# qdrant/quantization

Hardware: AMD Instinct MI355X
Metric: scored vectors/sec, 10Mx768 u8 dot (higher is better)
Workload: dtype u8; 1 GPU; 10000000 x 768 store: f32 U[0,1) -> scalar u8 (dot); per step: encode_query + score_all over the shard; quantizer=u8, rows_per_gpu=10000000, dim=768, distance=dot, exchange=scores, gather_group=1, launch=single rank, world_size_seen=1, encode_ahead=False, total_rows=10000000, queries=16

## Files before the change

quantization_amd/csrc/common.cpp:

```cpp
#include "common.hpp"

#include <sys/stat.h>

#include <cerrno>
#include <cmath>
#include <cstdlib>
#include <algorithm>
#include <atomic>
#include <fstream>
#include <mutex>
#include <vector>

namespace qamd {

static thread_local std::string g_last_error;
static thread_local int g_device = 0;

std::string &last_error() { return g_last_error; }

qamd_status fail(qamd_status st, const char *fmt, ...) {
    char buf[1024];
    va_list ap;
    va_start(ap, fmt);
    vsnprintf(buf, sizeof buf, fmt, ap);
    va_end(ap);
    g_last_error = buf;
    return st;
}

int current_device() { return g_device; }

int device_count() {
    static std::atomic<int> cached{-1};
    int n = cached.load(std::memory_order_relaxed);
    if (n > 0) return n;
    n = 0;
    if (hipGetDeviceCount(&n) != hipSuccess || n <= 0) {
        (void)hipGetLastError();
        return 0;
    }
    cached.store(n, std::memory_order_relaxed);
    return n;
}

DeviceGuard::DeviceGuard(int device) {
    const int n = device_count();
    if (n <= 0) {
        st_ = fail(QAMD_ERR_DEVICE, "no HIP device is visible; this library has no CPU fallback");
        return;
    }
    if (device < 0 || device >= n) {
        st_ = fail(QAMD_ERR_ARGUMENTS, "device %d out of range (have %d)", device, n);
        return;
    }
    hipError_t e = hipGetDevice(&prev_);
    if (e == hipSuccess && prev_ != device) {
        e = hipSetDevice(device);
        switched_ = e == hipSuccess;
    }
    if (e != hipSuccess) st_ = fail(QAMD_ERR_DEVICE, "cannot select device %d: %s", device, hipGetErrorString(e));
}

DeviceGuard::~DeviceGuard() {
    if (switched_) (void)hipSetDevice(prev_);
}

qamd_status DevBuf::alloc(size_t n, bool zero) {
    release();
    if (n == 0) n = 16;
    QAMD_HIP(hipMalloc(&ptr, n));
    bytes = n;
    if (zero) {
        QAMD_HIP(hipMemsetAsync(ptr, 0, n, nullptr));
        QAMD_HIP(hipStreamSynchronize(nullptr));
    }
    return QAMD_OK;
}

qamd_status DevBuf::alloc_zero_tail(size_t n, size_t keep) {
    QAMD_TRY(alloc(n, false));
    if (keep < bytes) {
        QAMD_HIP(hipMemsetAsync(static_cast<char *>(ptr) + keep, 0, bytes - keep, nullptr));
        QAMD_HIP(hipStreamSynchronize(nullptr));
    }
    return QAMD_OK;
}

void DevBuf::release() {
    if (ptr) (void)hipFree(ptr);
    ptr = nullptr;
    bytes = 0;
}

qamd_status grow_copy(const DevBuf &old, size_t n, size_t keep, DevBuf &out) {
    if (keep > n || keep > old.bytes) return fail(QAMD_ERR_ARGUMENTS, "grow_copy: keeps %zu of %zu bytes in %zu", keep, old.bytes, n);
    QAMD_TRY(out.alloc_zero_tail(n, keep));
    if (keep) {
        QAMD_HIP(hipMemcpyAsync(out.ptr, old.ptr, keep, hipMemcpyDeviceToDevice, nullptr));
        QAMD_HIP(hipStreamSynchronize(nullptr));
    }
    return QAMD_OK;
}

namespace {
struct QueryBufCache {
    struct Entry { void *ptr; size_t bytes; int dev; };
    std::mutex m;
    std::vector<Entry> free_list;
};
QueryBufCache &query_cache() {
    static QueryBufCache *c = new QueryBufCache;
    return *c;
}
constexpr size_t kQueryCacheEntries = 64;
}

qamd_status query_buf_get(size_t bytes, DevBuf &out) {
    out.release();
    int dev = 0;
    QAMD_HIP(hipGetDevice(&dev));
    {
        QueryBufCache &c = query_cache();
        std::lock_guard<std::mutex> lk(c.m);
        for (size_t i = 0; i < c.free_list.size(); i++) {
            if (c.free_list[i].dev == dev && c.free_list[i].bytes == bytes) {
                out.ptr = c.free_list[i].ptr;
                out.bytes = bytes;
                c.free_list[i] = c.free_list.back();
                c.free_list.pop_back();
                return QAMD_OK;
            }
        }
    }
    return out.alloc(bytes, true);
}

void query_buf_put(DevBuf &buf, bool idle) {
    if (!buf.ptr) return;
    hipPointerAttribute_t attr{};
    if (idle && hipPointerGetAttributes(&attr, buf.ptr) == hipSuccess) {
        QueryBufCache &c = query_cache();
        std::lock_guard<std::mutex> lk(c.m);
        if (c.free_list.size() < kQueryCacheEntries) {
            c.free_list.push_back({buf.ptr, buf.bytes, attr.device});
            buf.ptr = nullptr;
            buf.bytes = 0;
            return;
        }
    } else if (idle) {
        (void)hipGetLastError();
    }
    buf.release();
}

qamd_status StreamBuf::alloc(size_t n, hipStream_t s, bool zero) {
    release();
    static std::once_flag once[64];
    int dev = 0;
    if (hipGetDevice(&dev) == hipSuccess && dev >= 0 && dev < 64) {
        std::call_once(once[dev], [dev] {
            hipMemPool_t pool = nullptr;
            if (hipDeviceGetDefaultMemPool(&pool, dev) == hipSuccess && pool) {
                uint64_t keep = ~0ull;
                (void)hipMemPoolSetAttribute(pool, hipMemPoolAttrReleaseThreshold, &keep);
            }
        });
    }
    if (n == 0) n = 16;
    stream = s;
    QAMD_HIP(hipMallocAsync(&ptr, n, s));
    bytes = n;
    if (zero) QAMD_HIP(hipMemsetAsync(ptr, 0, n, s));
    return QAMD_OK;
}

void StreamBuf::release() {
    if (ptr) (void)hipFreeAsync(ptr, stream);
    ptr = nullptr;
    bytes = 0;
}

ReadyEvent::~ReadyEvent() {
    if (ev) (void)hipEventDestroy(ev);
}

qamd_status ReadyEvent::record(hipStream_t s) {
    if (!ev) QAMD_HIP(hipEventCreateWithFlags(&ev, hipEventDisableTiming));
    QAMD_HIP(hipEventRecord(ev, s));
    stream = s;
    set = true;
    return QAMD_OK;
}

bool ReadyEvent::complete() const {
    if (!set || !ev) return true;
    if (hipEventQuery(ev) == hipSuccess) return true;
    (void)hipGetLastError();
    return false;
}

qamd_status ReadyEvent::wait(hipStream_t consumer) const {
    if (!set || consumer == stream) return QAMD_OK;
    hipStreamCaptureStatus cap = hipStreamCaptureStatusNone;
    if (hipStreamIsCapturing(consumer, &cap) != hipSuccess) (void)hipGetLastError();
    if (cap == hipStreamCaptureStatusNone) {
        if (hipEventQuery(ev) == hipSuccess) return QAMD_OK;
        (void)hipGetLastError();
    }
    QAMD_HIP(hipStreamWaitEvent(consumer, ev, 0));
    return QAMD_OK;
}

qamd_status copy_in(void *dev_dst, const void *src, qamd_mem src_mem, size_t bytes, hipStream_t s) {
    if (bytes == 0) return QAMD_OK;
    if (src_mem == QAMD_MEM_DEVICE) {
        QAMD_HIP(hipMemcpyAsync(dev_dst, src, bytes, hipMemcpyDeviceToDevice, s));
    } else {
        QAMD_HIP(hipMemcpyAsync(dev_dst, src, bytes, hipMemcpyHostToDevice, s));
        QAMD_HIP(hipStreamSynchronize(s));
    }
    return QAMD_OK;
}

qamd_status copy_out(void *dst, qamd_mem dst_mem, const void *dev_src, size_t bytes, hipStream_t s) {
    if (bytes == 0) return QAMD_OK;
    if (dst_mem == QAMD_MEM_DEVICE) {
        QAMD_HIP(hipMemcpyAsync(dst, dev_src, bytes, hipMemcpyDeviceToDevice, s));
    } else {
        QAMD_HIP(hipMemcpyAsync(dst, dev_src, bytes, hipMemcpyDeviceToHost, s));
        QAMD_HIP(hipStreamSynchronize(s));
    }
    return QAMD_OK;
}

qamd_status local_view(const void *src, qamd_mem mem, size_t bytes, DevBuf &stage, hipStream_t s, const void **out,
                       bool *staged) {
    *out = src;
    *staged = false;
    if (bytes == 0) return QAMD_OK;
    bool remote = false;
    if (mem == QAMD_MEM_DEVICE && device_count() > 1) {
        hipPointerAttribute_t attr{};
        int dev = 0;
        if (hipPointerGetAttributes(&attr, src) == hipSuccess && hipGetDevice(&dev) == hipSuccess)
            remote = attr.device != dev;
        else
            (void)hipGetLastError();
    }
    if (mem == QAMD_MEM_DEVICE && !remote) return QAMD_OK;
    if (stage.bytes < bytes) QAMD_TRY(stage.alloc(bytes));
    QAMD_HIP(hipMemcpyAsync(stage.ptr, src, bytes, mem == QAMD_MEM_HOST ? hipMemcpyHostToDevice : hipMemcpyDefault, s));
    if (mem == QAMD_MEM_HOST) QAMD_HIP(hipStreamSynchronize(s));
    *out = stage.ptr;
    *staged = true;
    return QAMD_OK;
}

namespace {

constexpr int kMaxDevices = 64;

struct ThreadWs {
    void *ptr = nullptr;
    size_t bytes = 0;
    hipEvent_t done = nullptr;
    bool in_flight = false;
    uint64_t tags[3] = {0, 0, 0};
};

struct ThreadState {
    HostScratch scratch;
    bool scratch_tried = false;
    hipEvent_t query_read = nullptr;
    bool query_pending = false;
    std::vector<ThreadWs> ws;

    ThreadWs &at(int dev, ThreadWsSlot slot) {
        const size_t need = (size_t)(dev + 1) * WS_SLOTS;
        if (ws.size() < need) ws.resize(need);
        return ws[(size_t)dev * WS_SLOTS + slot];
    }

    void release() {
        int prev = -1;
        const bool have_prev = hipGetDevice(&prev) == hipSuccess;
        bool moved = false;
        for (size_t i = 0; i < ws.size(); i++) {
            ThreadWs &w = ws[i];
            if (!w.ptr) continue;
            const int dev = (int)(i / WS_SLOTS);
            if (hipSetDevice(dev) == hipSuccess) {
                moved = true;
                (void)hipFree(w.ptr);
                if (w.done) (void)hipEventDestroy(w.done);
            }
            w = ThreadWs{};
        }
        ws.clear();
        if (moved && have_prev) (void)hipSetDevice(prev);
        if (query_pending && query_read) (void)hipEventSynchronize(query_read);
        if (query_read) (void)hipEventDestroy(query_read);
        query_read = nullptr;
        query_pending = false;
        if (scratch.host) (void)hipHostFree(scratch.host);
        scratch = HostScratch{};
        scratch_tried = false;
        (void)hipGetLastError();
    }

    ~ThreadState() { release(); }
};

ThreadState &thread_state() {
    static thread_local ThreadState st;
    return st;
}

}

HostScratch host_scratch() {
    ThreadState &ts = thread_state();
    if (!ts.scratch_tried) {
        ts.scratch_tried = true;
        void *p = nullptr, *d = nullptr;
        if (hipHostMalloc(&p, kHostScratchWords * 4, hipHostMallocMapped | hipHostMallocPortable) == hipSuccess) {
            if (hipHostGetDevicePointer(&d, p, 0) == hipSuccess) {
                ts.scratch.host = static_cast<uint32_t *>(p);
                ts.scratch.dev = static_cast<uint32_t *>(d);
            } else {
                (void)hipHostFree(p);
            }
        }
    }
    return ts.scratch;
}

float *host_query_acquire(size_t n_floats, const float **dev_view) {
    if (n_floats > kHostQueryWords) return nullptr;
    const HostScratch hs = host_scratch();
    if (!hs.host) return nullptr;
    ThreadState &ts = thread_state();
    if (ts.query_pending) {
        if (hipEventSynchronize(ts.query_read) != hipSuccess) return nullptr;
        ts.query_pending = false;
    }
    if (!ts.query_read && hipEventCreateWithFlags(&ts.query_read, hipEventDisableTiming) != hipSuccess) {
        ts.query_read = nullptr;
        return nullptr;
    }
    *dev_view = reinterpret_cast<const float *>(hs.dev + kHostQueryAt);
    return reinterpret_cast<float *>(hs.host + kHostQueryAt);
}

void host_query_release(hipStream_t s) {
    ThreadState &ts = thread_state();
    if (ts.query_read && hipEventRecord(ts.query_read, s) == hipSuccess) ts.query_pending = true;
}

qamd_status thread_ws_acquire(ThreadWsSlot slot, size_t bytes, hipStream_t s, void **out, uint64_t **tags) {
    int dev = 0;
    QAMD_HIP(hipGetDevice(&dev));
    if (dev < 0 || dev >= kMaxDevices) return fail(QAMD_ERR_DEVICE, "device index %d not supported", dev);
    ThreadWs &w = thread_state().at(dev, slot);
    if (bytes == 0) bytes = 16;
    if (w.bytes < bytes) {
        if (w.ptr) {
            (void)hipFree(w.ptr);
            w.ptr = nullptr;
        }
        w.bytes = 0;
        w.in_flight = false;
        w.tags[0] = w.tags[1] = w.tags[2] = 0;
        const size_t want = bytes + bytes / 4;
        QAMD_HIP(hipMalloc(&w.ptr, want));
        w.bytes = want;
    }
    hipStreamCaptureStatus cap = hipStreamCaptureStatusNone;
    if (w.in_flight && hipStreamIsCapturing(s, &cap) != hipSuccess) (void)hipGetLastError();
    if (w.in_flight && cap == hipStreamCaptureStatusNone) {
        const hipError_t q = hipEventQuery(w.done);
        if (q == hipErrorNotReady) {
            (void)hipGetLastError();
            QAMD_HIP(hipStreamWaitEvent(s, w.done, 0));
        } else if (q != hipSuccess) {
            return fail(QAMD_ERR_DEVICE, "workspace hand-off: hipEventQuery failed: %s", hipGetErrorString(q));
        } else {
            w.in_flight = false;
        }
    }
    *out = w.ptr;
    if (tags) *tags = w.tags;
    return QAMD_OK;
}

void thread_ws_release(ThreadWsSlot slot, hipStream_t s, bool synced) {
    int dev = 0;
    if (hipGetDevice(&dev) != hipSuccess || dev < 0 || dev >= kMaxDevices) return;
    ThreadWs &w = thread_state().at(dev, slot);
    if (synced) {
        w.in_flight = false;
        return;
    }
    hipStreamCaptureStatus cap = hipStreamCaptureStatusNone;
    if (hipStreamIsCapturing(s, &cap) != hipSuccess) (void)hipGetLastError();
    if (cap != hipStreamCaptureStatusNone) return;
    w.in_flight = false;
    if (!w.done && hipEventCreateWithFlags(&w.done, hipEventDisableTiming) != hipSuccess) {
        w.done = nullptr;
        (void)hipGetLastError();
        (void)hipStreamSynchronize(s);
        return;
    }
    if (hipEventRecord(w.done, s) == hipSuccess) w.in_flight = true;
    else (void)hipStreamSynchronize(s);
}

void thread_release_all() { thread_state().release(); }

const DeviceInfo &device_info() {
    static DeviceInfo info[kMaxDevices];
    static std::atomic<uint64_t> known{0};
    int dev = 0;
    if (hipGetDevice(&dev) != hipSuccess || dev < 0 || dev >= kMaxDevices) dev = 0;
    if (!(known.load(std::memory_order_acquire) & (1ull << dev))) {
        hipDeviceProp_t p;
        if (hipGetDeviceProperties(&p, dev) == hipSuccess && p.multiProcessorCount > 0)
            info[dev].cu_count = p.multiProcessorCount;
        static const uint64_t forced = dev_env_u64("QAMD_DEV_CU_COUNT", 0);
        if (forced) info[dev].cu_count = (int)std::min<uint64_t>(forced, 1024);
        known.fetch_or(1ull << dev, std::memory_order_acq_rel);
    }
    return info[dev];
}

std::string json_f32(float v) {
    if (!std::isfinite(v)) return "null";
    std::string sign = std::signbit(v) ? "-" : "";
    if (v == 0.0f) return sign + "0.0";
    char buf[64];
    const double a = std::fabs((double)v);
    for (int p = 0; p <= 8; p++) {
        snprintf(buf, sizeof buf, "%.*e", p, a);
        if (strtof(buf, nullptr) == std::fabs(v)) break;
    }
    std::string digits;
    const char *e = strchr(buf, 'e');
    for (const char *c = buf; c < e; c++)
        if (*c != '.') digits += *c;
    const int exp10 = atoi(e + 1), length = (int)digits.size();
    const int kk = exp10 + 1, k = kk - length;
    if (0 <= k && kk <= 13) return sign + digits + std::string((size_t)k, '0') + ".0";
    if (0 < kk && kk <= 13) return sign + digits.substr(0, (size_t)kk) + "." + digits.substr((size_t)kk);
    if (-6 < kk && kk <= 0) return sign + "0." + std::string((size_t)(-kk), '0') + digits;
    if (length == 1) return sign + digits + "e" + std::to_string(kk - 1);
    return sign + digits.substr(0, 1) + "." + digits.substr(1) + "e" + std::to_string(kk - 1);
}

bool read_file(const char *path, std::string &out) {
    std::ifstream f(path, std::ios::binary);
    if (!f) return false;
    f.seekg(0, std::ios::end);
    std::streamoff n = f.tellg();
    f.seekg(0, std::ios::beg);
    out.resize((size_t)n);
    if (n > 0) f.read(&out[0], n);
    return bool(f) || f.eof();
}

static bool write_file(const char *path, const void *data, size_t bytes) {
    std::ofstream f(path, std::ios::binary | std::ios::trunc);
    if (!f) return false;
    if (bytes) f.write(static_cast<const char *>(data), (std::streamsize)bytes);
    f.flush();
    return bool(f);
}

static void make_parent_dirs(const char *path) {
    std::string p(path);
    size_t pos = p.find_last_of('/');
    if (pos == std::string::npos || pos == 0) return;
    std::string dir = p.substr(0, pos);
    for (size_t i = 1; i <= dir.size(); i++) {
        if (i == dir.size() || dir[i] == '/') {
            std::string sub = dir.substr(0, i);
            if (mkdir(sub.c_str(), 0777) != 0 && errno != EEXIST) return;
        }
    }
}

qamd_status save_file(const char *path, const void *data, size_t bytes) {
    make_parent_dirs(path);
    if (!write_file(path, data, bytes)) return fail(QAMD_ERR_IO, "cannot write %s", path);
    return QAMD_OK;
}

qamd_status load_rows_file(const char *data_path, uint64_t expected, std::string &bytes) {
    if (!read_file(data_path, bytes)) return fail(QAMD_ERR_IO, "cannot read %s", data_path);
    if (bytes.size() != expected)
        return fail(QAMD_ERR_IO, "Loaded storage size %zu is not equal to expected size %llu", bytes.size(),
                    (unsigned long long)expected);
    return QAMD_OK;
}

qamd_status count_mismatch(uint64_t got, uint64_t want) {
    return fail(QAMD_ERR_ARGUMENTS, "Vector count %llu does not match vector parameters count %llu", (unsigned long long)got,
// ... 99 lines not shown
```

quantization_amd/csrc/common.hpp:

```cpp
#pragma once

#include <hip/hip_runtime.h>

#include <algorithm>
#include <atomic>
#include <mutex>
#include <cstdarg>
#include <cstdint>
#include <cstdlib>
#include <cstdio>
#include <cstring>
#include <string>
#include <vector>

#include "json.hpp"

#include "../../include/quantization_amd.h"

namespace qamd {

std::string &last_error();
qamd_status fail(qamd_status st, const char *fmt, ...) __attribute__((format(printf, 2, 3)));

#define QAMD_HIP(expr)                                                                      \
    do {                                                                                    \
        hipError_t _e = (expr);                                                             \
        if (_e != hipSuccess)                                                               \
            return ::qamd::fail(QAMD_ERR_DEVICE, "%s failed: %s (%s:%d)", #expr,            \
                                hipGetErrorString(_e), __FILE__, __LINE__);                 \
    } while (0)

#define QAMD_TRY(expr)                    \
    do {                                  \
        qamd_status _s = (expr);          \
        if (_s != QAMD_OK) return _s;     \
    } while (0)

int current_device();
int device_count();

class DeviceGuard {
  public:
    explicit DeviceGuard(int device);
    ~DeviceGuard();
    DeviceGuard(const DeviceGuard &) = delete;
    DeviceGuard &operator=(const DeviceGuard &) = delete;
    qamd_status status() const { return st_; }

  private:
    int prev_ = -1;
    bool switched_ = false;
    qamd_status st_ = QAMD_OK;
};
#define QAMD_ON_DEVICE(dev)                  \
    ::qamd::DeviceGuard _qamd_dev_guard(dev); \
    QAMD_TRY(_qamd_dev_guard.status())

inline const char *dev_env(const char *name) {
#ifdef QAMD_DEV
    return getenv(name);
#else
    (void)name;
    return nullptr;
#endif
}
inline uint64_t dev_env_u64(const char *name, uint64_t dflt) {
    const char *e = dev_env(name);
    if (!e || !*e) return dflt;
    char *end = nullptr;
    const unsigned long long v = strtoull(e, &end, 10);
    return (*end == 0 && v > 0) ? (uint64_t)v : dflt;
}
inline uint64_t stage_bytes(uint64_t dflt) {
    static const uint64_t v = dev_env_u64("QAMD_DEV_STAGE_BYTES", 0);
    return v ? v : dflt;
}
inline bool host_whole_allowed() {
    static const bool on = [] { const char *e = dev_env("QAMD_DEV_HOST_WHOLE"); return !(e && e[0] == '0'); }();
    return on;
}
inline bool u8_packed_allowed() {
    static const bool on = [] { const char *e = dev_env("QAMD_DEV_U8_PACKED"); return !(e && e[0] == '0'); }();
    return on;
}
inline uint64_t pq_planar_max_rows() {
    static const uint64_t v = dev_env_u64("QAMD_DEV_PQ_PLANAR_ROWS", 1ull << 28);
    return v;
}
inline uint64_t pq_skew_max_rows() {
    static const uint64_t v = dev_env_u64("QAMD_DEV_PQ_SKEW_ROWS", 1ull << 30);
    return v;
}

class DeviceOnce {
  public:
    template <class F> qamd_status run(F &&setup) {
        int dev = 0;
        if (hipGetDevice(&dev) != hipSuccess || dev < 0 || dev > 63) return setup();
        const uint64_t bit = 1ull << dev;
        if (done_.load(std::memory_order_acquire) & bit) return QAMD_OK;
        std::lock_guard<std::mutex> g(mu_);
        if (done_.load(std::memory_order_relaxed) & bit) return QAMD_OK;
        const qamd_status st = setup();
        if (st == QAMD_OK) done_.fetch_or(bit, std::memory_order_release);
        return st;
    }

  private:
    std::atomic<uint64_t> done_{0};
    std::mutex mu_;
};
#define QAMD_LDS_OPT_IN(kernel, bytes)                                                                            \
    do {                                                                                                          \
        static ::qamd::DeviceOnce _qamd_once;                                                                     \
        QAMD_TRY(_qamd_once.run([]() -> qamd_status {                                                             \
            QAMD_HIP(hipFuncSetAttribute(reinterpret_cast<const void *>(kernel),                                  \
                                         hipFuncAttributeMaxDynamicSharedMemorySize, (int)(bytes)));              \
            return QAMD_OK;                                                                                       \
        }));                                                                                                      \
    } while (0)

struct DevBuf {
    void *ptr = nullptr;
    size_t bytes = 0;
    DevBuf() = default;
    DevBuf(const DevBuf &) = delete;
    DevBuf &operator=(const DevBuf &) = delete;
    DevBuf(DevBuf &&o) noexcept : ptr(o.ptr), bytes(o.bytes) { o.ptr = nullptr; o.bytes = 0; }
    DevBuf &operator=(DevBuf &&o) noexcept {
        if (this != &o) {
            release();
            ptr = o.ptr;
            bytes = o.bytes;
            o.ptr = nullptr;
            o.bytes = 0;
        }
        return *this;
    }
    ~DevBuf() { release(); }
    qamd_status alloc(size_t n, bool zero = false);
    qamd_status alloc_zero_tail(size_t n, size_t keep);
    void release();
    template <typename T> T *as() const { return static_cast<T *>(ptr); }
};

qamd_status grow_copy(const DevBuf &old, size_t n, size_t keep, DevBuf &out);

qamd_status query_buf_get(size_t bytes, DevBuf &out);
void query_buf_put(DevBuf &buf, bool idle);

inline hipStream_t as_stream(void *s) { return static_cast<hipStream_t>(s); }

struct StreamBuf {
    void *ptr = nullptr;
    size_t bytes = 0;
    hipStream_t stream = nullptr;
    StreamBuf() = default;
    StreamBuf(const StreamBuf &) = delete;
    StreamBuf &operator=(const StreamBuf &) = delete;
    ~StreamBuf() { release(); }
    qamd_status alloc(size_t n, hipStream_t s, bool zero = false);
    void release();
    template <typename T> T *as() const { return static_cast<T *>(ptr); }
};

struct ReadyEvent {
    hipEvent_t ev = nullptr;
    hipStream_t stream = nullptr;
    bool set = false;
    ReadyEvent() = default;
    ReadyEvent(const ReadyEvent &) = delete;
    ReadyEvent &operator=(const ReadyEvent &) = delete;
    ~ReadyEvent();
    qamd_status record(hipStream_t s);
    qamd_status wait(hipStream_t consumer) const;
    bool complete() const;
};

qamd_status copy_in(void *dev_dst, const void *src, qamd_mem src_mem, size_t bytes, hipStream_t s);
qamd_status copy_out(void *dst, qamd_mem dst_mem, const void *dev_src, size_t bytes, hipStream_t s);

constexpr size_t kHostQueryWords = 12288;
constexpr size_t kHostDoneAt = 2048 + 8;
constexpr size_t kHostQueryAt = 2048 + 16;
constexpr size_t kHostScratchWords = kHostQueryAt + kHostQueryWords;
struct HostScratch {
    uint32_t *host = nullptr;
    uint32_t *dev = nullptr;
};
HostScratch host_scratch();
float *host_query_acquire(size_t n_floats, const float **dev_view);
void host_query_release(hipStream_t s);

enum ThreadWsSlot { WS_SCORES = 0, WS_SELECT = 1, WS_PARTIAL = 2, WS_FUSED = 3, WS_SMALL = 4, WS_RESCORE = 5, WS_ROW_LUT = 6, WS_SLOTS = 7 };
qamd_status thread_ws_acquire(ThreadWsSlot slot, size_t bytes, hipStream_t s, void **out,
                              uint64_t **tags = nullptr);
void thread_ws_release(ThreadWsSlot slot, hipStream_t s, bool synced = false);
void thread_release_all();

qamd_status local_view(const void *src, qamd_mem mem, size_t bytes, DevBuf &stage, hipStream_t s, const void **out,
                       bool *staged);

template <class Consume>
qamd_status for_each_staged_piece(const float *batch, qamd_mem batch_mem, uint64_t n_rows, uint64_t dim, uint64_t piece_rows,
                                  DevBuf &stage, hipStream_t s, Consume &&consume) {
    for (uint64_t r = 0; r < n_rows; r += piece_rows) {
        const uint64_t nr = std::min(piece_rows, n_rows - r);
        const void *src = nullptr;
        bool staged = false;
        QAMD_TRY(local_view(batch + r * dim, batch_mem, nr * dim * 4, stage, s, &src, &staged));
        QAMD_TRY(consume(static_cast<const float *>(src), r, nr));
        if (staged) QAMD_HIP(hipStreamSynchronize(s));
    }
    return QAMD_OK;
}
qamd_status count_mismatch(uint64_t got, uint64_t want);
template <class Encoder> void abort_encoder(Encoder *e) {
    if (!e) return;
    DeviceGuard g(e->device);
    (void)hipStreamSynchronize(e->stream);
    delete e;
}
qamd_status check_row_range(uint64_t first_row, uint64_t n_rows, uint64_t count);
qamd_status check_upsert(uint64_t first_row, uint64_t n_rows, uint64_t count, const void *data, uint64_t dim);
constexpr uint64_t kRowPad = 1024;
inline uint64_t padded_rows_of(uint64_t capacity) { return (capacity + kRowPad - 1) / kRowPad * kRowPad + kRowPad; }
inline uint64_t upsert_capacity(uint64_t needed, uint64_t capacity) { return std::max(needed, capacity + capacity / 2); }

struct DeviceInfo {
    int cu_count = 256;
};
const DeviceInfo &device_info();

inline uint64_t round_up(uint64_t v, uint64_t m) { return (v + m - 1) / m * m; }

std::string json_f32(float v);
bool read_file(const char *path, std::string &out);
qamd_status save_file(const char *path, const void *data, size_t bytes);
qamd_status load_rows_file(const char *data_path, uint64_t expected, std::string &bytes);
qamd_status read_metadata(const char *meta_path, JsonValue &root);

qamd_status refuse_u8_flags(const qamd_vector_parameters *vp);

const char *distance_name(int d);
bool parse_distance(const std::string &s, int &d);
std::string vector_parameters_json(const qamd_vector_parameters &vp);
bool parse_vector_parameters(const JsonValue &obj, qamd_vector_parameters &vp, std::string &err);

}
```

quantization_amd/csrc/u8.hip:

```cpp
#include <algorithm>
#include <cmath>
#include <cstdlib>
#include <memory>
#include <type_traits>
#include <vector>

#include "common.hpp"
#include "lists.hpp"
#include "multi_reduce.hpp"
#include "topk.hpp"
#include "topk_device.hpp"
#include "rescore.hpp"
#include "rotate_blocks.hpp"
#include "u8_internal.hpp"

#pragma clang fp contract(off)

using namespace qamd;
using namespace qamd::rot;

namespace {

constexpr int kBlock = 256;
constexpr int kScanBlock = 512;
// ... 783 lines not shown
        if (lane == 0 && zk != 0xFFFFFFFFu) {
            const unsigned long long key = tile_key + zk;
            if (key < __builtin_nontemporal_load(first_zero)) atomicMin(first_zero, key);
        }
    }
}

template <int ITERS , bool FAST ,
          bool FOUR = false >
__global__ __launch_bounds__(kScanBlock) void quantize16_kernel(
    const float *__restrict__ data, uint64_t n_rows, uint32_t dim, uint32_t actual_dim, float alpha,
    float offset, int distance, int invert, uint32_t *__restrict__ codes32, float *__restrict__ offsets,
    uint64_t row0) {
    const float r_alpha = 1.0f / alpha;
    const int lane = threadIdx.x & 63, sub = lane & 15, rslot = lane >> 4;
    const uint64_t wave = ((uint64_t)blockIdx.x * kScanBlock + threadIdx.x) >> 6;
    if (wave * 4 >= n_rows) return;
    const uint64_t r = wave * 4 + rslot;
    const bool row_ok = r < n_rows;
    const uint64_t rc = row_ok ? r : n_rows - 1;
    const float *src = data + rc * dim;
    const float4 *src4 = reinterpret_cast<const float4 *>(src);
    const uint32_t dwords = actual_dim / 4, f4 = dim / 4;
    uint32_t *dst = codes32 + (row0 + rc) * dwords;
    const float placeholder = (distance == QAMD_DOT) ? 0.0f : offset;
    const uint32_t pad_code = f32_to_code<FOUR>(placeholder, alpha, offset);
    const uint32_t pad_dword = pad_code * 0x01010101u;
    uint32_t s1 = 0, s2 = 0;
    constexpr int DEPTH = ITERS ? ITERS : 4;
    for (uint32_t d0 = sub; d0 < dwords; d0 += 16 * DEPTH) {
        float4 f[DEPTH];
#pragma unroll
        for (int j = 0; j < DEPTH; j++) {
            const uint32_t d = d0 + 16 * j;
            f[j] = d < f4 ? ld_nt(src4 + d) : make_float4(0.0f, 0.0f, 0.0f, 0.0f);
        }
#pragma unroll
        for (int j = 0; j < DEPTH; j++) {
            const uint32_t d = d0 + 16 * j;
            if (d >= dwords) break;
            uint32_t packed;
            if (d < f4) {
                if (FAST) {
                    packed = f32x4_to_u8x4_fast(f[j], alpha, offset, r_alpha);
                } else {
                    packed = f32_to_code<FOUR>(f[j].x, alpha, offset) | (f32_to_code<FOUR>(f[j].y, alpha, offset) << 8) |
                             (f32_to_code<FOUR>(f[j].z, alpha, offset) << 16) | (f32_to_code<FOUR>(f[j].w, alpha, offset) << 24);
                }
                s1 = __builtin_amdgcn_udot4(packed, 0x01010101u, s1, false);
                s2 = __builtin_amdgcn_udot4(packed, packed, s2, false);
            } else {
                packed = pad_dword;
                s1 += 4 * pad_code;
                s2 += 4 * pad_code * pad_code;
            }
            if (row_ok) __builtin_nontemporal_store(packed, dst + d);
        }
        if (ITERS) break;
    }
    s1 = group_sum<16>(s1);
    s2 = group_sum<16>(s2);
    if (sub == 0 && row_ok) {
        float vo;
        const float D = (float)actual_dim;
        if (distance == QAMD_DOT) {
            float sum = (float)s1;
            if (s1 >= (1u << 24)) {
                sum = 0.0f;
                for (uint32_t j = 0; j < actual_dim; j++)
                    sum += (float)(j < dim ? f32_to_code<FOUR>(src[j], alpha, offset) : pad_code);
            }
            vo = D * offset * offset + sum * alpha * offset;
        } else if (distance == QAMD_L1) {
            vo = 0.0f;
        } else {
            float sum = (float)s2;
            if (s2 >= (1u << 24)) {
                sum = 0.0f;
                for (uint32_t j = 0; j < actual_dim; j++) {
                    const float c = (float)(j < dim ? f32_to_code<FOUR>(src[j], alpha, offset) : pad_code);
                    sum += c * c;
                }
            }
            vo = D * offset * offset + sum * alpha * alpha;
        }
        offsets[row0 + r] = invert ? -vo : vo;
    }
}

__global__ __launch_bounds__(kBlock) void quantize_kernel(
    const float *__restrict__ data, uint64_t n_rows, uint32_t dim, uint32_t actual_dim, float alpha,
    float offset, int distance, int invert, uint32_t *__restrict__ codes32 ,
    float *__restrict__ offsets, uint64_t row0, int four) {
    const int lane = threadIdx.x & 63;
    const uint64_t wave = ((uint64_t)blockIdx.x * kBlock + threadIdx.x) >> 6;
    const uint64_t n_waves = ((uint64_t)gridDim.x * kBlock) >> 6;
    const float placeholder = (distance == QAMD_DOT) ? 0.0f : offset;
    const uint32_t pad_code = f32_to_code(placeholder, alpha, offset, four);
    const uint32_t dwords = actual_dim / 4;
    for (uint64_t r = wave; r < n_rows; r += n_waves) {
        const float *src = data + r * dim;
        uint32_t *dst = codes32 + (row0 + r) * dwords;
        uint32_t s1 = 0, s2 = 0;
        for (uint32_t d = lane; d < dwords; d += 64) {
            uint32_t packed = 0;
#pragma unroll
            for (int b = 0; b < 4; b++) {
                uint32_t j = d * 4 + b;
                uint32_t c = j < dim ? f32_to_code(src[j], alpha, offset, four) : pad_code;
                packed |= c << (8 * b);
                s1 += c;
                s2 += c * c;
            }
            dst[d] = packed;
        }
#pragma unroll
        for (int m = 1; m < 64; m <<= 1) {
            s1 += __shfl_xor(s1, m, 64);
            s2 += __shfl_xor(s2, m, 64);
        }
        if (lane == 0) {
            float vo;
            const float D = (float)actual_dim;
            if (distance == QAMD_DOT) {
                float s = (float)s1;
                if (s1 >= (1u << 24)) {
                    s = 0.0f;
                    for (uint32_t j = 0; j < actual_dim; j++)
                        s += (float)(j < dim ? f32_to_code(src[j], alpha, offset, four) : pad_code);
                }
                vo = D * offset * offset + s * alpha * offset;
            } else if (distance == QAMD_L1) {
                vo = 0.0f;
            } else {
                float s = (float)s2;
                if (s2 >= (1u << 24)) {
                    s = 0.0f;
                    for (uint32_t j = 0; j < actual_dim; j++) {
                        float c = (float)(j < dim ? f32_to_code(src[j], alpha, offset, four) : pad_code);
                        s += c * c;
                    }
                }
                vo = D * offset * offset + s * alpha * alpha;
            }
            offsets[row0 + r] = invert ? -vo : vo;
        }
    }
}

constexpr int kQuant4Bit = 2;
__device__ __forceinline__ uint32_t rot_quant4(const float (&v)[4], float alpha, float offset, float r_alpha, int fast) {
    const float4 f = make_float4(v[0], v[1], v[2], v[3]);
    if (fast == kQuant4Bit)
        return f32_to_u4(f.x, alpha, offset) | (f32_to_u4(f.y, alpha, offset) << 8) | (f32_to_u4(f.z, alpha, offset) << 16) |
               (f32_to_u4(f.w, alpha, offset) << 24);
    if (fast) return f32x4_to_u8x4_fast(f, alpha, offset, r_alpha);
    return f32_to_u8(f.x, alpha, offset) | (f32_to_u8(f.y, alpha, offset) << 8) | (f32_to_u8(f.z, alpha, offset) << 16) |
           (f32_to_u8(f.w, alpha, offset) << 24);
}
__device__ __forceinline__ float rot_row_offset(uint32_t dim, float alpha, float offset, int distance, int invert, uint32_t s1,
                                                float sum2) {
    const float D = (float)dim;
    float vo;
    if (distance == QAMD_DOT) {
        const float sum = (float)s1;
        vo = D * offset * offset + sum * alpha * offset;
    } else {
        vo = D * offset * offset + sum2 * alpha * alpha;
    }
    return invert ? -vo : vo;
}
__device__ __forceinline__ void rot_minmax_commit(float mn, float mx, unsigned long long zk, uint64_t slot_id, int lane,
                                                  uint32_t *__restrict__ slots, uint64_t base_values,
                                                  unsigned long long *__restrict__ first_zero) {
#pragma unroll
    for (int m = 1; m < 64; m <<= 1) {
        float o = __shfl_xor(mn, m, 64);
        mn = o < mn ? o : mn;
        o = __shfl_xor(mx, m, 64);
        mx = o > mx ? o : mx;
        const unsigned long long z = __shfl_xor(zk, m, 64);
        zk = z < zk ? z : zk;
    }
    if (lane == 0) {
        uint32_t *slot = slots + (slot_id & (kMinmaxSlots - 1)) * kMinmaxSlotStride;
        const uint32_t kmn = f32_order_key(mn), kmx = f32_order_key(mx);
        if (kmn < __builtin_nontemporal_load(slot)) atomicMin(slot, kmn);
        if (kmx > __builtin_nontemporal_load(slot + 1)) atomicMax(slot + 1, kmx);
        if ((mn == 0.0f || mx == 0.0f) && zk != kNoZero) atomicMin(first_zero, (base_values << 1) + zk);
    }
}

struct RotMinmaxSink : RotSink {
    uint32_t dim;
    float c;
    uint32_t *slots;
    uint64_t base_values;
    unsigned long long *first_zero;
    struct State {
        float mn = 3.40282347e+38f, mx = -3.40282347e+38f;
        unsigned long long zk = kNoZero;
        uint32_t z = 0xFFFFFFFFu;
    };
    __device__ void chunk(State &st, uint64_t, uint32_t ch, int, const float (&y)[4], uint32_t &) const {
#pragma unroll
        for (int e = 0; e < 4; e++) {
            const float v = __fmul_rn(y[e], c);
            st.mn = v < st.mn ? v : st.mn;
            st.mx = v > st.mx ? v : st.mx;
            if (v == 0.0f && st.z == 0xFFFFFFFFu) st.z = ((ch * 4 + e) << 1) | (__float_as_uint(v) >> 31);
        }
    }
    __device__ void row_end(State &st, uint64_t r) const {
        if (st.z != 0xFFFFFFFFu && st.zk == kNoZero) st.zk = ((r * dim) << 1) + st.z;
        st.z = 0xFFFFFFFFu;
    }
    template <int K> __device__ void row_wave(State &st, uint64_t r, int, const uint32_t (&)[K]) const { row_end(st, r); }
    __device__ void row_lds(State &st, uint64_t r, uint32_t *) const { row_end(st, r); }
    __device__ void finish(State &st, uint64_t slot_id, int lane) const {
        rot_minmax_commit(st.mn, st.mx, st.zk, slot_id, lane, slots, base_values, first_zero);
    }
};

struct RotQuantizeSink : RotSink {
    uint32_t dim;
    float c, alpha, offset;
    int fast, distance, invert;
    uint32_t *codes32;
    float *offsets;
    uint64_t row0;
    struct State {
        uint32_t s1 = 0, s2 = 0;
    };
    __device__ void chunk(State &st, uint64_t r, uint32_t ch, int, const float (&y)[4], uint32_t &keep) const {
        const float v[4] = {__fmul_rn(y[0], c), __fmul_rn(y[1], c), __fmul_rn(y[2], c), __fmul_rn(y[3], c)};
        const uint32_t p = rot_quant4(v, alpha, offset, 1.0f / alpha, fast);
        st.s1 = __builtin_amdgcn_udot4(p, 0x01010101u, st.s1, false);
        st.s2 = __builtin_amdgcn_udot4(p, p, st.s2, false);
        __builtin_nontemporal_store(p, codes32 + (row0 + r) * (dim / 4) + ch);
        keep = p;
    }
    __device__ bool replays(uint32_t s2) const { return distance == QAMD_L2 && s2 >= (1u << 24); }
    __device__ static void add_squares(float &sum2, uint32_t p) {
#pragma unroll
        for (int e = 0; e < 4; e++) {
            const float cf = (float)((p >> (8 * e)) & 0xFFu);
            sum2 += cf * cf;
        }
    }
    __device__ void wave_sums(State &st) const {
#pragma unroll
        for (int m = 1; m < 64; m <<= 1) {
            st.s1 += __shfl_xor(st.s1, m, 64);
            st.s2 += __shfl_xor(st.s2, m, 64);
        }
    }
    template <int K> __device__ void row_wave(State &st, uint64_t r, int lane, const uint32_t (&kept)[K]) const {
        wave_sums(st);
        const uint32_t s1 = (uint32_t)__builtin_amdgcn_readfirstlane((int)st.s1);
        const uint32_t s2 = (uint32_t)__builtin_amdgcn_readfirstlane((int)st.s2);
        float sum2 = (float)s2;
        if (replays(s2)) {
            sum2 = 0.0f;
#pragma unroll
            for (int k = 0; k < K; k++)
                for (uint32_t l = 0; l < 64 && (uint32_t)(k * 64) + l < dim / 4; l++)
                    add_squares(sum2, (uint32_t)__builtin_amdgcn_readlane((int)kept[k], (int)l));
        }
        if (lane == 0) offsets[row0 + r] = rot_row_offset(dim, alpha, offset, distance, invert, s1, sum2);
        st = State();
    }
    __device__ void row_lds(State &st, uint64_t r, uint32_t *row_u) const {
        wave_sums(st);
        __syncthreads();
        if ((threadIdx.x & 63) == 0) {
            row_u[(threadIdx.x >> 6) * 4 + 1] = st.s1;
            row_u[(threadIdx.x >> 6) * 4 + 2] = st.s2;
        }
        __syncthreads();
        if (threadIdx.x == 0) {
            uint32_t s1 = 0, s2 = 0;
            for (int w = 0; w < kRotThreads / 64; w++) s1 += row_u[w * 4 + 1], s2 += row_u[w * 4 + 2];
            float sum2 = (float)s2;
            if (replays(s2)) {
                sum2 = 0.0f;
                for (uint32_t ch = 0; ch < dim / 4; ch++) add_squares(sum2, row_u[ch * 4]);
            }
            offsets[row0 + r] = rot_row_offset(dim, alpha, offset, distance, invert, s1, sum2);
        }
        st = State();
    }
};

struct RotValuesSink : RotSink {
    uint32_t dim;
    float c;
    float *out;
    __device__ void chunk(State &, uint64_t r, uint32_t ch, int, const float (&y)[4], uint32_t &) const {
        reinterpret_cast<float4 *>(out + r * dim)[ch] =
            make_float4(__fmul_rn(y[0], c), __fmul_rn(y[1], c), __fmul_rn(y[2], c), __fmul_rn(y[3], c));
    }
};

__global__ __launch_bounds__(64) void encode_query_kernel(const float *__restrict__ query,
                                                         uint32_t qdim, uint32_t actual_dim,
                                                         float alpha, float offset, int distance,
                                                         int invert, uint8_t *__restrict__ qbuf, int four) {
    const int lane = threadIdx.x;
    const float placeholder = (distance == QAMD_DOT) ? 0.0f : offset;
    const uint32_t pad_code = f32_to_code(placeholder, alpha, offset, four);
    uint8_t *codes = qbuf + 16;
    uint32_t s1 = 0, s2 = 0;
    for (uint32_t j = lane; j < actual_dim; j += 64) {
        uint32_t c = j < qdim ? f32_to_code(query[j], alpha, offset, four) : pad_code;
        codes[j] = (uint8_t)c;
        s1 += c;
        s2 += c * c;
    }
#pragma unroll
    for (int m = 1; m < 64; m <<= 1) {
        s1 += __shfl_xor(s1, m, 64);
        s2 += __shfl_xor(s2, m, 64);
    }
    if (lane == 0) {
        float off;
        if (distance == QAMD_DOT) {
            float s = (float)s1;
            if (s1 >= (1u << 24)) {
                s = 0.0f;
                for (uint32_t j = 0; j < actual_dim; j++)
                    s += (float)(j < qdim ? f32_to_code(query[j], alpha, offset, four) : pad_code);
            }
            off = s * alpha * offset;
        } else if (distance == QAMD_L1) {
            off = 0.0f;
        } else {
            float s = (float)s2;
            if (s2 >= (1u << 24)) {
                s = 0.0f;
                for (uint32_t j = 0; j < actual_dim; j++) {
                    float c = (float)(j < qdim ? f32_to_code(query[j], alpha, offset, four) : pad_code);
                    s += c * c;
                }
            }
            off = s * alpha * alpha;
        }
        *reinterpret_cast<float *>(qbuf) = invert ? -off : off;
    }
}

__global__ __launch_bounds__(64) void encode_queries_kernel(const float *__restrict__ queries, uint32_t qdim,
                                                           uint32_t actual_dim, float alpha, float offset,
                                                           int distance, int invert, uint8_t *__restrict__ codes_out,
                                                           uint32_t code_pitch, float *__restrict__ offsets_out, int four) {
    const int lane = threadIdx.x;
    const float *query = queries + (size_t)blockIdx.x * qdim;
    uint8_t *codes = codes_out + (size_t)blockIdx.x * code_pitch;
    const float placeholder = (distance == QAMD_DOT) ? 0.0f : offset;
    const uint32_t pad_code = f32_to_code(placeholder, alpha, offset, four);
    uint32_t s1 = 0, s2 = 0;
    for (uint32_t j = lane; j < actual_dim; j += 64) {
        uint32_t c = j < qdim ? f32_to_code(query[j], alpha, offset, four) : pad_code;
        codes[j] = (uint8_t)c;
        s1 += c;
        s2 += c * c;
    }
#pragma unroll
    for (int m = 1; m < 64; m <<= 1) {
        s1 += __shfl_xor(s1, m, 64);
        s2 += __shfl_xor(s2, m, 64);
    }
    if (lane == 0) {
        float off;
        if (distance == QAMD_DOT) {
            float s = (float)s1;
            if (s1 >= (1u << 24)) {
                s = 0.0f;
                for (uint32_t j = 0; j < actual_dim; j++)
                    s += (float)(j < qdim ? f32_to_code(query[j], alpha, offset, four) : pad_code);
            }
            off = s * alpha * offset;
        } else if (distance == QAMD_L1) {
            off = 0.0f;
        } else {
            float s = (float)s2;
            if (s2 >= (1u << 24)) {
                s = 0.0f;
                for (uint32_t j = 0; j < actual_dim; j++) {
                    float c = (float)(j < qdim ? f32_to_code(query[j], alpha, offset, four) : pad_code);
                    s += c * c;
                }
            }
            off = s * alpha * alpha;
        }
        offsets_out[blockIdx.x] = invert ? -off : off;
    }
}

__global__ __launch_bounds__(kBlock) void split_rows_kernel(const uint32_t *__restrict__ rows32,
                                                           uint64_t n_rows, uint32_t row_dwords,
                                                           uint32_t *__restrict__ codes32,
                                                           float *__restrict__ offsets) {
    const uint64_t total = n_rows * row_dwords;
    const uint64_t stride = (uint64_t)gridDim.x * kBlock;
    for (uint64_t t = (uint64_t)blockIdx.x * kBlock + threadIdx.x; t < total; t += stride) {
        uint64_t r = t / row_dwords;
        uint32_t k = (uint32_t)(t - r * row_dwords);
        uint32_t w = rows32[t];
        if (k == 0)
            offsets[r] = __uint_as_float(w);
        else
            codes32[r * (row_dwords - 1) + (k - 1)] = w;
    }
}

__global__ __launch_bounds__(kBlock) void join_rows_kernel(const uint32_t *__restrict__ codes32,
                                                          const float *__restrict__ offsets,
                                                          uint64_t n_rows, uint32_t row_dwords,
                                                          uint32_t *__restrict__ rows32) {
    const uint64_t total = n_rows * row_dwords;
    const uint64_t stride = (uint64_t)gridDim.x * kBlock;
    for (uint64_t t = (uint64_t)blockIdx.x * kBlock + threadIdx.x; t < total; t += stride) {
        uint64_t r = t / row_dwords;
        uint32_t k = (uint32_t)(t - r * row_dwords);
        rows32[t] = k == 0 ? __float_as_uint(offsets[r]) : codes32[r * (row_dwords - 1) + (k - 1)];
    }
}

template <class IMG>
__global__ __launch_bounds__(kBlock) void u8_pack_image_kernel(const uint4 *__restrict__ codes, uint64_t r0, uint64_t n_rows,
                                                               uint32_t row_chunks, uint32_t pchunks,
                                                               uint4 *__restrict__ packed, uint32_t *__restrict__ bad) {
    const uint64_t total = n_rows * pchunks, stride = (uint64_t)gridDim.x * kBlock;
    uint32_t seen = 0;
    for (uint64_t t = (uint64_t)blockIdx.x * kBlock + threadIdx.x; t < total; t += stride) {
        const uint64_t r = r0 + t / pchunks;
        const uint32_t j = (uint32_t)(t % pchunks);
        packed[((r / kPackBlockRows) * pchunks + j) * kPackBlockRows + r % kPackBlockRows] =
            IMG::chunk(codes + r * row_chunks, j, row_chunks, pchunks, seen);
    }
    if (bad && (seen & IMG::kNoCode)) atomicOr(bad, 1u);
}

int grid_for(uint64_t work_items, uint64_t per_block, int blocks_per_cu) {
    uint64_t want = (work_items + per_block - 1) / per_block;
    uint64_t cap = (uint64_t)device_info().cu_count * blocks_per_cu;
    if (want < 1) want = 1;
    return (int)(want > cap ? cap : want);
}

float host_multiplier(float alpha, int distance, int invert) {
    float m = distance == QAMD_DOT ? alpha * alpha : distance == QAMD_L1 ? alpha : -2.0f * alpha * alpha;
    return invert ? -m : m;
}

uint64_t actual_dim_of(uint64_t dim) { return dim + (16 - dim % 16) % 16; }

float rot_scale_of(uint32_t B) {
    const int lg = __builtin_ctz(B);
    return std::ldexp((lg & 1) ? 0.70710678118654752440f : 1.0f, -(lg / 2));
}
template <class SINK> qamd_status launch_rot_u8(SINK sink, const float *src, uint64_t n, uint64_t dim, hipStream_t s) {
    if (n == 0) return QAMD_OK;
    const uint32_t B = (uint32_t)rot_block(dim);
    sink.dim = (uint32_t)dim, sink.c = rot_scale_of(B);
    launch_rot(sink, src, n, (uint32_t)dim, (uint32_t)dim, B, s);
    QAMD_HIP(hipGetLastError());
    return QAMD_OK;
}

qamd_status launch_rot_minmax(const float *src, uint64_t n, uint64_t dim, uint32_t *slots, uint64_t base_values,
                              unsigned long long *first_zero, hipStream_t s) {
    RotMinmaxSink sink;
    sink.slots = slots, sink.base_values = base_values, sink.first_zero = first_zero;
    return launch_rot_u8(sink, src, n, dim, s);
}
qamd_status launch_rot_values(const float *src, uint64_t n, uint64_t dim, float *out, hipStream_t s) {
    RotValuesSink sink;
    sink.out = out;
    return launch_rot_u8(sink, src, n, dim, s);
}
bool rot_dim_ok(uint64_t dim) { return dim != 0 && dim % kRotBlockMin == 0 && dim <= kRotMaxDim; }

}


namespace {

qamd_status alloc_store(qamd_u8 *h) {
    h->capacity = h->count;
    h->padded_rows = padded_rows_of(h->capacity);
    h->row_chunks = (uint32_t)(h->meta.actual_dim / 16);
    QAMD_TRY(h->codes.alloc_zero_tail(h->padded_rows * h->meta.actual_dim, h->count * h->meta.actual_dim));
    QAMD_TRY(h->offsets.alloc_zero_tail(h->padded_rows * sizeof(float), h->count * sizeof(float)));
    return QAMD_OK;
}

U8Image u8_image_of(uint32_t rc, bool four_bit, int distance) {
    if (distance == QAMD_L1 || rc > 128 || rc < (four_bit ? 2u : 8u)) return U8Image{};
    if (four_bit) return U8Image{U8_IMAGE_NIBBLE, (rc + 1) / 2, rc};
    return U8Image{U8_IMAGE_7BIT, rc - rc / 8, rc / 8};
}

qamd_status launch_pack(const qamd_u8 *h, uint64_t r0, uint64_t n_rows, uint32_t *bad, hipStream_t s) {
    const auto kernel = h->image.kind == U8_IMAGE_NIBBLE ? u8_pack_image_kernel<Image4> : u8_pack_image_kernel<Image7>;
    hipLaunchKernelGGL(kernel, dim3(grid_for(n_rows * h->image.chunks, kBlock, 8)), dim3(kBlock), 0, s, h->codes.as<uint4>(),
                       r0, n_rows, h->row_chunks, h->image.chunks, h->packed.as<uint4>(), bad);
    QAMD_HIP(hipGetLastError());
    return QAMD_OK;
}

qamd_status build_packed(qamd_u8 *h, hipStream_t s) {
    h->packed.release();
    h->packed_rows.release();
    h->image = U8Image{};
    const U8Image im = u8_image_of(h->row_chunks, h->four_bit, h->meta.vector_parameters.distance_type);
    if (!u8_packed_allowed() || h->count == 0 || !im.kind) return QAMD_OK;
    const uint64_t bytes = h->padded_rows * im.chunks * 16;
    size_t free_b = 0, total_b = 0;
    if (hipMemGetInfo(&free_b, &total_b) != hipSuccess || free_b < 2 * bytes) {
        (void)hipGetLastError();
        return QAMD_OK;
    }
    DevBuf bad;
    const std::string err = last_error();
    if (h->packed.alloc_zero_tail(bytes, h->count / kPackBlockRows * kPackBlockRows * im.chunks * 16) != QAMD_OK ||
        bad.alloc(sizeof(uint32_t), true) != QAMD_OK) {
        (void)hipGetLastError();
        last_error() = err;
        h->packed.release();
        return QAMD_OK;
    }
    h->image = im;
    uint32_t high = 1;
    const qamd_status st = [&]() -> qamd_status {
        QAMD_TRY(launch_pack(h, 0, h->count, bad.as<uint32_t>(), s));
        QAMD_HIP(hipMemcpyAsync(&high, bad.ptr, sizeof(high), hipMemcpyDeviceToHost, s));
        QAMD_HIP(hipStreamSynchronize(s));
        return QAMD_OK;
    }();
    if (st != QAMD_OK || high) {
        h->packed.release();
        h->image = U8Image{};
    }
    return st;
}

struct ScanEpi {
    float diff = 0.0f;
    int mode = EPI_POINT;
    uint64_t rows = 0;
};
inline uint64_t scan_rows(const qamd_u8 *h, const ScanEpi &e) { return e.rows ? e.rows : h->count; }

template <class F> void with_bool(bool b, F &&f) {
    if (b) f(std::true_type{});
    else f(std::false_type{});
}
template <class F> void with_epi(int mode, F &&f) {
    if (mode == EPI_POINT) f(std::integral_constant<int, EPI_POINT>{});
    else f(std::integral_constant<int, EPI_INTERNAL>{});
}

template <bool IS_L1> struct ScanLaunch {
    template <int G, int ITERS, int UNROLL>
    static void go(const qamd_u8 *h, const uint4 *qc, const float *qo, float *out, const TopkFilter *filt, hipStream_t s,
                   const ScanEpi &e) {
        constexpr int TILE = (64 / G) * UNROLL;
        const uint64_t waves = (scan_rows(h, e) + TILE - 1) / TILE;
        const unsigned grid = (unsigned)((waves + kScanBlock / 64 - 1) / (kScanBlock / 64));
        with_bool(h->row_chunks == (uint32_t)(G * ITERS), [&](auto ex) {
            with_bool(filt != nullptr, [&](auto fi) {
                with_epi(e.mode, [&](auto epi) {
                    hipLaunchKernelGGL((u8_scan_kernel<G, ITERS, UNROLL, IS_L1, ex, fi, epi>), dim3(grid), dim3(kScanBlock), 0,
                                       s, h->codes.as<uint4>(), h->offsets.as<float>(), qc, qo, h->meta.multiplier,
                                       (uint32_t)scan_rows(h, e), h->row_chunks, out, filt ? *filt : TopkFilter{}, e.diff);
                });
            });
        });
    }
};

uint32_t blocked_split(uint64_t count) {
    const uint64_t blocks = (count + kPackBlockRows - 1) / kPackBlockRows;
    const uint64_t want = (uint64_t)device_info().cu_count * 16;
    uint32_t split = 1;
    while (split < 8 && blocks * split < want) split *= 2;
    return split;
}

void launch_scan_image(const qamd_u8 *h, const uint4 *qc, const float *qo, float *out, const TopkFilter *filt,
                       hipStream_t s, const ScanEpi &e) {
    const uint64_t n_rows = scan_rows(h, e);
    const uint32_t split = blocked_split(n_rows), blocks_per_wg = (kScanBlock / 64) / split;
    const uint64_t blocks = (n_rows + kPackBlockRows - 1) / kPackBlockRows;
    const unsigned grid = (unsigned)((blocks + blocks_per_wg - 1) / blocks_per_wg);
    h->last_scan_split.store((int)split, std::memory_order_relaxed);
    with_bool(h->image.kind == U8_IMAGE_NIBBLE, [&](auto nibble) {
        using IMG = std::conditional_t<nibble, Image4, Image7>;
        with_bool(filt != nullptr, [&](auto fi) {
            with_epi(e.mode, [&](auto epi) {
                hipLaunchKernelGGL((u8_scan_image_kernel<IMG, fi, epi>), dim3(grid), dim3(kScanBlock), 0, s,
                                   h->packed.as<uint4>(), h->offsets.as<float>(), qc, qo, h->meta.multiplier, (uint32_t)n_rows,
                                   h->image.chunks, h->image.aux, split, out, filt ? *filt : TopkFilter{}, e.diff);
            });
        });
    });
}

template <bool IS_L1>
bool launch_scan(const qamd_u8 *h, const uint4 *qc, const float *qo, float *out, const TopkFilter *filt,
                 hipStream_t s, const ScanEpi &e) {
    using L = ScanLaunch<IS_L1>;
    h->last_scan_packed.store(h->image.kind, std::memory_order_relaxed);
    if (h->image.kind) return launch_scan_image(h, qc, qo, out, filt, s, e), true;
    const uint32_t rc = h->row_chunks;
    if (rc == 1) return L::template go<1, 1, 4>(h, qc, qo, out, filt, s, e), true;
    if (rc == 2) return L::template go<2, 1, 4>(h, qc, qo, out, filt, s, e), true;
    if (rc <= 4) return L::template go<4, 1, 8>(h, qc, qo, out, filt, s, e), true;
    if (rc <= 8) return L::template go<8, 1, 8>(h, qc, qo, out, filt, s, e), true;
    switch ((rc + 15) / 16) {
// ... 1582 lines not shown
```

Measured before the change: 10.04 billion vectors/s.

## Vectorize query encode loads/stores and defer ready-event recording on null stream

The query encode kernel now loads four floats per lane as float4 (with a scalar fallback for misaligned input), unrolls several trips, and packs four codes into a 32-bit word store instead of writing bytes one at a time. Separately, ReadyEvent skips creating and recording a HIP event when recorded on the null stream, deferring the event record until a consumer on another stream actually waits. This targets per-query encode latency and per-call event API overhead, at the cost of more complex tail handling and a mutex on every event operation.

```diff
diff --git a/quantization_amd/csrc/common.cpp b/quantization_amd/csrc/common.cpp
--- a/quantization_amd/csrc/common.cpp
+++ b/quantization_amd/csrc/common.cpp
@@ -185,15 +185,33 @@
 }
 
 qamd_status ReadyEvent::record(hipStream_t s) {
+    std::lock_guard<std::mutex> lk(mu);
+    if (s == nullptr) {
+        QAMD_HIP(hipGetDevice(&device));
+        stream = s;
+        set = true;
+        pending = true;
+        return QAMD_OK;
+    }
     if (!ev) QAMD_HIP(hipEventCreateWithFlags(&ev, hipEventDisableTiming));
     QAMD_HIP(hipEventRecord(ev, s));
     stream = s;
     set = true;
+    pending = false;
     return QAMD_OK;
 }
 
 bool ReadyEvent::complete() const {
-    if (!set || !ev) return true;
+    std::lock_guard<std::mutex> lk(mu);
+    if (!set) return true;
+    if (pending) {
+        DeviceGuard on(device);
+        if (on.status() != QAMD_OK) return false;
+        if (hipStreamQuery(nullptr) == hipSuccess) return true;
+        (void)hipGetLastError();
+        return false;
+    }
+    if (!ev) return true;
     if (hipEventQuery(ev) == hipSuccess) return true;
     (void)hipGetLastError();
     return false;
@@ -201,6 +219,15 @@
 
 qamd_status ReadyEvent::wait(hipStream_t consumer) const {
     if (!set || consumer == stream) return QAMD_OK;
+    {
+        std::lock_guard<std::mutex> lk(mu);
+        if (pending) {
+            QAMD_ON_DEVICE(device);
+            if (!ev) QAMD_HIP(hipEventCreateWithFlags(&ev, hipEventDisableTiming));
+            QAMD_HIP(hipEventRecord(ev, stream));
+            pending = false;
+        }
+    }
     hipStreamCaptureStatus cap = hipStreamCaptureStatusNone;
     if (hipStreamIsCapturing(consumer, &cap) != hipSuccess) (void)hipGetLastError();
     if (cap == hipStreamCaptureStatusNone) {
diff --git a/quantization_amd/csrc/common.hpp b/quantization_amd/csrc/common.hpp
--- a/quantization_amd/csrc/common.hpp
+++ b/quantization_amd/csrc/common.hpp
@@ -165,9 +165,12 @@
 };
 
 struct ReadyEvent {
-    hipEvent_t ev = nullptr;
+    mutable hipEvent_t ev = nullptr;
     hipStream_t stream = nullptr;
     bool set = false;
+    int device = 0;
+    mutable bool pending = false;
+    mutable std::mutex mu;
     ReadyEvent() = default;
     ReadyEvent(const ReadyEvent &) = delete;
     ReadyEvent &operator=(const ReadyEvent &) = delete;
diff --git a/quantization_amd/csrc/u8.hip b/quantization_amd/csrc/u8.hip
--- a/quantization_amd/csrc/u8.hip
+++ b/quantization_amd/csrc/u8.hip
@@ -1109,6 +1109,53 @@
     }
 };
 
+constexpr int kEncodeTrip = 4;
+template <bool VEC>
+__device__ __forceinline__ void encode_query_codes(const float *__restrict__ query, uint32_t qdim, uint32_t actual_dim,
+                                                   float alpha, float offset, uint32_t pad_code, int four,
+                                                   uint32_t *__restrict__ codes32, uint32_t &s1, uint32_t &s2) {
+    const uint32_t j_rest = qdim & ~3u;
+    for (uint32_t j0 = threadIdx.x * 4; j0 < actual_dim; j0 += 64 * 4 * kEncodeTrip) {
+        float v[kEncodeTrip][4];
+        float rest[3] = {0.0f, 0.0f, 0.0f};
+#pragma unroll
+        for (int k = 0; k < kEncodeTrip; k++) {
+            const uint32_t j = j0 + (uint32_t)k * 256;
+            if (VEC) {
+                float4 t = make_float4(0.0f, 0.0f, 0.0f, 0.0f);
+                if (j + 4 <= qdim) t = *reinterpret_cast<const float4 *>(query + j);
+                v[k][0] = t.x, v[k][1] = t.y, v[k][2] = t.z, v[k][3] = t.w;
+            } else {
+#pragma unroll
+                for (int e = 0; e < 4; e++) {
+                    v[k][e] = 0.0f;
+                    if (j + e < qdim) v[k][e] = query[j + e];
+                }
+            }
+        }
+        if (VEC && j_rest >= j0 && j_rest < j0 + 256 * kEncodeTrip && (j_rest - j0) % 256 == 0) {
+#pragma unroll
+            for (int e = 0; e < 3; e++)
+                if (j_rest + e < qdim) rest[e] = query[j_rest + e];
+        }
+#pragma unroll
+        for (int k = 0; k < kEncodeTrip; k++) {
+            const uint32_t j = j0 + (uint32_t)k * 256;
+            if (j >= actual_dim) break;
+            uint32_t word = 0;
+#pragma unroll
+            for (int e = 0; e < 4; e++) {
+                const float x = (VEC && e < 3 && j == j_rest) ? rest[e] : v[k][e];
+                const uint32_t c = j + e < qdim ? f32_to_code(x, alpha, offset, four) : pad_code;
+                word |= c << (8 * e);
+                s1 += c;
+                s2 += c * c;
+            }
+            codes32[j / 4] = word;
+        }
+    }
+}
+
 __global__ __launch_bounds__(64) void encode_query_kernel(const float *__restrict__ query,
                                                          uint32_t qdim, uint32_t actual_dim,
                                                          float alpha, float offset, int distance,
@@ -1116,14 +1163,12 @@
     const int lane = threadIdx.x;
     const float placeholder = (distance == QAMD_DOT) ? 0.0f : offset;
     const uint32_t pad_code = f32_to_code(placeholder, alpha, offset, four);
-    uint8_t *codes = qbuf + 16;
+    uint32_t *codes32 = reinterpret_cast<uint32_t *>(qbuf + 16);
     uint32_t s1 = 0, s2 = 0;
-    for (uint32_t j = lane; j < actual_dim; j += 64) {
-        uint32_t c = j < qdim ? f32_to_code(query[j], alpha, offset, four) : pad_code;
-        codes[j] = (uint8_t)c;
-        s1 += c;
-        s2 += c * c;
-    }
+    if ((reinterpret_cast<uintptr_t>(query) & 15) == 0)
+        encode_query_codes<true>(query, qdim, actual_dim, alpha, offset, pad_code, four, codes32, s1, s2);
+    else
+        encode_query_codes<false>(query, qdim, actual_dim, alpha, offset, pad_code, four, codes32, s1, s2);
 #pragma unroll
     for (int m = 1; m < 64; m <<= 1) {
         s1 += __shfl_xor(s1, m, 64);
```

After: 10.10 billion vectors/s (median of 6 runs). No clear change (+0.6%).
